# keillernogueira/dynamic-rs-segmentation

Hardware: AMD Instinct MI355X
Metric: training patches/sec dilated_grsl_rate8 64x64x5 (higher is better)
Workload: dtype f32; 1 GPU; dilated_grsl_rate8 (Dilated8Pooling) training step, single_fixed 64x64, 5-band synthetic 2048x2048 tile, global batch 128 (crop+augment+normalise, fwd, loss, bwd, momentum, confusion); global_batch=128, patch=64, bands=5, classes=6, parallelism=dp1, sync_bn=True, rccl_ranks_observed=1

## Files before the change

dynamic-rs-segmentation_amd/_lib.py:

```python
import ctypes as C
import os

_HERE = os.path.dirname(os.path.abspath(__file__))
LIB_PATH = os.path.join(_HERE, "libdrs_hip.so")
DEV_LIB_PATH = os.path.join(_HERE, "libdrs_hip_dev.so")

_p, _i, _f, _d = C.c_void_p, C.c_int, C.c_float, C.c_double
_sz, _u64 = C.c_size_t, C.c_ulonglong

SIGNATURES = {
    "drs_conv_mtile": (_i, [_i]),
    "drs_conv_forward": (_i, [_p, _i, _i, _i, _i, _i, _p, _p, _i, _i, _i, _i, _i, _p, _i, _i, _i, _p, _p]),
    "drs_conv_workspace_floats": (_sz, [_i]),
    "drs_conv_halo_skip": (_i, [_i, _i, _i, _i, _i, _i, _i]),
    "drs_conv_executed_ksteps": (_i, [_i, _i, _i, _i, _i, _i, _i, _p, _p]),
    "drs_conv_forward_ws": (_i, [_p, _i, _i, _i, _i, _i, _p, _p, _i, _i, _i, _i, _i, _p, _i, _i, _i, _p, _p, _sz, _p]),
    "drs_conv_wgrad_splits": (_i, [_i, _i, _i, _i, _i]),
    "drs_conv_wgrad": (_i, [_p, _i, _i, _i, _i, _i, _p, _i, _i, _i, _i, _i, _i, _i, _i, _i, _p, _p, _p]),
    "drs_filter_flip_transpose": (_i, [_p, _p, _i, _i, _i, _p]),
    "drs_filter_pad_cin": (_i, [_p, _p, _i, _i, _i, _i, _p]),
    "drs_split_conv_mtile": (_i, [_i]),
    "drs_split_terms": (_i, [_p, _sz, _i, _p, _p]),
    "drs_filter_split": (_i, [_p, _i, _i, _i, _i, _i, _p, _p, _p]),
    "drs_conv_forward_split": (_i, [_p, _i, _i, _i, _i, _i, _p, _p, _i, _i, _i, _i, _i, _p, _i, _i, _i, _p, _i, _p]),
# ... 73 lines not shown
    "drs_net_receptive_field": (_i, [_p, C.POINTER(_i), C.POINTER(_i)]),
    "drs_net_receptive_field_gated": (_i, [_p, C.POINTER(_i), C.POINTER(_i)]),
    "drs_net_se_info": (_i, [_p, _i, C.c_char_p, _i, C.POINTER(_i), C.POINTER(_i), C.POINTER(_i)]),
    "drs_net_type_name": (_i, [_i, C.c_char_p, _i, C.POINTER(_i)]),
    "drs_net_num_variables": (_i, [_p]),
    "drs_net_variable_info": (_i, [_p, _i, C.c_char_p, _i, C.POINTER(_sz), C.POINTER(_sz), C.POINTER(_i), C.POINTER(_i)]),
    "drs_params_get": (_i, [_p, C.c_char_p, C.c_char_p, _p, _sz, _p]),
    "drs_params_set": (_i, [_p, C.c_char_p, C.c_char_p, _p, _sz, _p]),
    "drs_grad_buffer": (_i, [_p, C.POINTER(_p), C.POINTER(_sz)]),
    "drs_net_global_step": (C.c_longlong, [_p, C.c_longlong]),
    "drs_net_learning_rate": (_f, [_p, _f]),
    "drs_net_set_comm": (_i, [_p, _i, _i, _p, _p, _p]),
    "drs_rccl_bind_library": (_i, [C.c_char_p]),
    "drs_rccl_available": (_i, []),
    "drs_rccl_form": (_i, []),
    "drs_rccl_unique_id": (_i, [_p]),
    "drs_rccl_comm_create": (_i, [_i, _i, _p, C.POINTER(_p)]),
    "drs_rccl_comm_destroy": (_i, [_p]),
    "drs_rccl_all_reduce": (_i, [_p, _p, C.c_size_t, _i, _p]),
    "drs_net_set_rccl": (_i, [_p, _i, _i, _p, _p, _p]),
    "drs_train_step": (_i, [_p, _i, _i, _f, _i, _d, _p]),
    "drs_forward": (_i, [_p, _i, _i, _i, _i, _p]),
    "drs_apply_update": (_i, [_p, _f, _p]),
    "drs_forward_staged": (_i, [_p, _i, _i, _i, _p, _i, _i, _p]),
    "drs_net_se_gate_finish": (_i, [_p, _i, _d, _p]),
    "drs_net_set_two_streams": (_i, [_p, _i]),
    "drs_net_set_class_weights": (_i, [_p, _p, _i]),
    "drs_net_get_class_weights": (_i, [_p, _p, _i, C.POINTER(_i)]),
    "drs_net_set_focal_gamma": (_i, [_p, _f]),
    "drs_net_get_focal_gamma": (_i, [_p, C.POINTER(_f)]),
    "drs_net_timing": (_i, [_p, _i]),
    "drs_net_num_timing_kinds": (_i, []),
    "drs_net_timing_summary": (_i, [_p, _i, C.c_char_p, _i, C.POINTER(_i), C.POINTER(_d), C.POINTER(_d)]),
}
ALLREDUCE_FN = C.CFUNCTYPE(_i, _p, _p, _sz, _i, _i, _p)
WAIT_FN = C.CFUNCTYPE(_i, _p, _i, _p)
WANT_LOGITS, WITH_LABELS, USE_ACC_MASK, USE_LOSS_MASK, NO_UPDATE = 1, 2, 4, 8, 16


DEV_SIGNATURES = {
    "drs_debug_skip_taps": (_i, [_i]), "drs_debug_conv_variant": (_i, [_i]), "drs_debug_conv_wide192": (_i, [_i]),
    "drs_debug_conv_splitk": (_i, [_i]), "drs_debug_conv_hybrid": (_i, [_i]), "drs_debug_conv_sk_order": (_i, [_i]), "drs_debug_conv_prio": (_i, [_i]),
    "drs_debug_conv_sk_geometry": (_i, [_i, _i, _i, _p]), "drs_debug_conv_trace": (_i, [_p]), "drs_debug_conv_lpt": (_i, [_i]), "drs_debug_conv_order": (_i, [_i] * 7 + [_p, _i]),
    "drs_debug_conv_image_tiles": (_i, [_i]), "drs_debug_conv_order_image": (_i, [_i] * 7 + [_p, _i]),
    "drs_debug_wgrad_variant": (_i, [_i]), "drs_debug_wgrad_seg": (_i, [_i]), "drs_debug_wgrad_balance": (_i, [_i]), "drs_debug_wgrad_target": (_i, [_i]),
    "drs_debug_wgrad_len": (_i, [_i]), "drs_debug_wgrad_minchunks": (_i, [_i]), "drs_debug_wgrad_prio": (_i, [_i]), "drs_debug_cls_variant": (_i, [_i]), "drs_debug_slide_blocks": (_i, [_i]), "drs_debug_slide_minrows": (_i, [_i]), "drs_debug_slide_rowpad": (_i, [_i]), "drs_debug_chain_mode": (_i, [_i]), "drs_debug_jitter": (_i, [C.c_ulonglong]), "drs_debug_wg_stream_prio": (_i, [_i]), "drs_debug_reductions_on_chain": (_i, [_i]), "drs_debug_wgrad_schedule": (_i, [_i, _i, _i]), "drs_debug_variant": (_i, [_i]),
    "drs_debug_wgrad_cut": (_i, [_i] * 7 + [_p, _i, _p, _p]),
}


class DrsError(RuntimeError):
    pass


_lib = None
_dev = None


def _open(path, signatures):
    if not os.path.isfile(path):
        raise DrsError("HIP library not built: %s is missing (run dynamic-rs-segmentation_amd/csrc/build.sh "
                       "or __graft_entry__.build()); there is no CPU fallback" % path)
    import torch
    lib = C.CDLL(path)
    for name, (res, args) in signatures.items():
        fn = getattr(lib, name)
        fn.restype = res
        fn.argtypes = args
    return lib


def load():
    global _lib
    if _lib is None:
        _lib = _open(LIB_PATH, SIGNATURES)
    return _lib


class _Dev(object):
# ... 40 lines not shown
```

dynamic-rs-segmentation_amd/csrc/conv_mfma.hip:

```cpp
#include "drs_common.hpp"
#include <algorithm>
#include <cstdlib>
#include <map>
#include <mutex>
#include <numeric>
#include <tuple>
#include <vector>

namespace {

constexpr int BK = 32;
constexpr int LDA = BK + 4;

struct ConvArgs {
  const float* in; int S, P, ld_in, coff_in;
  int M;
  const float* w;
  const float* bias;
  float* out; int ld_out, coff_out;
  float* stats;
  int k, rate, pad, Cin, Cout;
  int accumulate;
  int skip_halo;
  float rcpS, rcpSS;
// ... 1210 lines not shown
  if (W > cap) {
    if (g_conv_splitk <= 0) return plain;
    W = cap; if (G < W || T == tiles) G = W;
  }
  return SkGeom{(int)G, (int)W, (int)T};
}

void conv_lpt_setup(ConvArgs& a, int BM, int mt, int nt, int W) {
  a.lpt_T = 0; a.lpt_ta = a.lpt_tb = a.lpt_P = 0;
  if (W || !g_conv_lpt || drs_g_skip_halo_taps == 0) return;
  const int S2 = a.S * a.S, T = S2 % BM == 0 ? S2 / BM : 0, nblk = mt * nt;
  if (T < 2 || BM % a.S != 0 || nblk % 8 != 0 || (nblk / 8) % (T * nt) != 0) return;
  const int rows = BM / a.S;
  auto full = [&](int t) {
    const int y0 = t * rows, y1 = y0 + rows - 1;
    const int lo = a.pad - y1 > 0 ? (a.pad - y1 + a.rate - 1) / a.rate : 0;
    int hi = (a.S - 1 - y0 + a.pad) / a.rate + 1;
    hi = hi < a.k ? hi : a.k;
    return lo == 0 && hi == a.k;
  };
  int ta = 0, tb = T;
  while (ta < T && !full(ta)) ++ta;
  while (tb > ta && !full(tb - 1)) --tb;
  bool ok = ta < tb;
  for (int t = ta; ok && t < tb; ++t) ok = full(t);
  if (ok && (ta > 0 || tb < T)) { a.lpt_T = T; a.lpt_ta = ta; a.lpt_tb = tb; a.lpt_P = nblk / 8 / (T * nt); a.skip_halo = 1; }
}

int g_conv_image_tiles = -1;

int conv_image_tiles_rule(int k, int rate, int cin, int cout, int B, int S) {
  if (B != 128 || S != 64) return 0;
  struct Row { int k, rate, cin, cout; };
  static const Row gains[] = {{4, 3, 64, 128},
                              {4, 4, 128, 128},
                              {3, 5, 128, 192}, {3, 5, 192, 128},
                              {3, 6, 192, 192},
                              {3, 7, 192, 256}, {3, 7, 256, 192},
                              {3, 8, 256, 256}};
  for (const Row& r : gains)
    if (r.k == k && r.rate == rate && r.cin == cin && r.cout == cout) return 7;
  return 0;
}

int conv_image_tiles_g(int B, int S, int k, int rate, int cin, int cout) {
  const int g = g_conv_image_tiles < 0 ? conv_image_tiles_rule(k, rate, cin, cout, B, S) : g_conv_image_tiles;
  if (g < 4 || g > 7 || k < 2 || cin < BK || cin % BK || g_conv_variant == 0) return 0;
  if (B % (1 << g) || S % (128 >> g)) return 0;
  return g;
}

inline int image_tile_taps(int mt, int S, int k, int rate, int pad, int g) {
  int y, x0, ul, uh, vl, vh;
  image_tile_pos(mt, S, g, y, x0);
  live_taps_image_tile(y, x0, 128 >> g, S, k, rate, pad, ul, uh, vl, vh);
  return (uh - ul) * (vh - vl);
}

std::vector<int> conv_image_order(int B, int S, int k, int rate, int pad, int g) {
  const int mt = B * S * S / 128;
  std::vector<int> taps(mt), sorted(mt), order(mt);
  for (int i = 0; i < mt; ++i) taps[i] = image_tile_taps(i, S, k, rate, pad, g);
  std::iota(sorted.begin(), sorted.end(), 0);
  std::stable_sort(sorted.begin(), sorted.end(), [&](int x, int y) { return taps[x] > taps[y]; });
  if (mt % 8) return sorted;
  const int per = mt / 8;
  for (int c = 0; c < 8; ++c)
    for (int j = 0; j < per; ++j) order[c * per + j] = sorted[j * 8 + c];
  return order;
}

const int* conv_image_order_device(int B, int S, int k, int rate, int pad, int g) {
  static std::mutex mu;
  static std::map<std::tuple<int, int, int, int, int, int, int>, const int*> cache;
  int dev = 0;
  if (hipGetDevice(&dev) != hipSuccess) return nullptr;
  std::lock_guard<std::mutex> lock(mu);
  const auto key = std::make_tuple(dev, B, S, k, rate, pad, g);
  const auto it = cache.find(key);
  if (it != cache.end()) return it->second;
  const std::vector<int> order = conv_image_order(B, S, k, rate, pad, g);
  int* d = nullptr;
  if (hipMalloc((void**)&d, order.size() * sizeof(int)) != hipSuccess) return nullptr;
  if (hipMemcpy(d, order.data(), order.size() * sizeof(int), hipMemcpyHostToDevice) != hipSuccess) { (void)hipFree(d); return nullptr; }
  cache[key] = d;
  return d;
}

template <int BM, int BN, int WM, int WN>
// ... 342 lines not shown
  const int mt = (int)((M + 127) / 128), nt = cout / bn;
  const int W = sk_geometry(mt * nt, k * k * (cin / 32), bn, drs_conv_workspace_floats(cout)).G;
  if (W) return 0;
  conv_lpt_setup(a, 128, mt, nt, 0);
  return a.skip_halo;
}

int drs_conv_executed_ksteps(int B, int S, int k, int rate, int pad_before, int cin, int cout, long long* executed, long long* total) {
  const long long M = (long long)B * S * S;
  if (B < 1 || S < 1 || M >= (1 << 24) || cout < 32 || cout % 32 || cin < 1 || k < 1 || rate < 1 || !executed || !total) return DRS_ERR_ARG;
  const int bn = pick_conv_tile(cout, cin), bm = bn >= 64 ? 128 : 256;
  const int mt = (int)((M + bm - 1) / bm), nt = cout / bn;
  const long long cpt = cin < 32 ? 1 : cin / 32;
  *total = *executed = cin < 32 ? (long long)mt * nt * ((k * k * cin + 31) / 32) : (long long)mt * nt * k * k * cpt;
  if (cin < 32 || cin % 32) return DRS_OK;
  const int g = conv_plain_image_g(B, S, k, rate, cin, cout);
  long long taps = 0;
  if (g) {
    if (drs_g_skip_halo_taps == 0) return DRS_OK;
    for (int i = 0; i < mt; ++i) taps += image_tile_taps(i, S, k, rate, pad_before, g);
  } else {
    if (!drs_conv_halo_skip(B, S, k, rate, pad_before, cin, cout)) return DRS_OK;
    for (int i = 0; i < mt; ++i) {
      const int p0 = i * bm, p1 = (int)(p0 + bm < M ? p0 + bm : M) - 1;
      int y0 = (p0 % (S * S)) / S, y1 = (p1 % (S * S)) / S;
      if (p0 / (S * S) != p1 / (S * S)) { y0 = 0; y1 = S - 1; }
      int lo = pad_before - y1 > 0 ? (pad_before - y1 + rate - 1) / rate : 0, hi = (S - 1 - y0 + pad_before) / rate + 1;
      hi = hi < k ? hi : k;
      if (lo >= hi) { lo = 0; hi = k; }
      taps += (hi - lo) * k;
    }
  }
  *executed = taps * nt * cpt;
  return DRS_OK;
}

int drs_conv_forward_ws(const float* in, int B, int S, int P, int ld_in, int coff_in, const float* w, const float* bias,
                        int k, int rate, int pad_before, int cin, int cout, float* out, int ld_out, int coff_out,
                        int accumulate, float* stats_partial, float* workspace, size_t workspace_floats, void* stream) {
  if (!in || !w || !out || (cin % 32 && cin != 8 && cin != 16) || cout % 32 || k < 1 || rate < 1 || P < pad_before) return DRS_ERR_ARG;
  if (B < 1 || S < 1 || cin < 8 || cout < 32 || pad_before < 0 || !drs_prod_below(1LL << 31, {k, k, cin, cout})) return DRS_ERR_ARG;
  if (coff_in < 0 || ld_in < coff_in + cin || coff_out < 0 || ld_out < coff_out + cout) return DRS_ERR_ARG;
  if (cin < 32 && (ld_in % 4 || coff_in % 4)) return DRS_ERR_ARG;
  if (accumulate && stats_partial) return DRS_ERR_ARG;
  if (P < (long long)(k - 1) * rate - pad_before) return DRS_ERR_ARG;
  const long long M = (long long)B * S * S;
  if (M <= 0 || M >= (1 << 24)) return DRS_ERR_ARG;
  if ((long long)B * (S + 2 * P) * (S + 2 * P) * ld_in >= (1LL << 30)) return DRS_ERR_ARG;
  ConvArgs a;
  a.in = in; a.S = S; a.P = P; a.ld_in = ld_in; a.coff_in = coff_in; a.M = (int)M;
  a.w = w; a.bias = bias; a.out = out; a.ld_out = ld_out; a.coff_out = coff_out; a.stats = stats_partial;
  a.k = k; a.rate = rate; a.pad = pad_before; a.Cin = cin; a.Cout = cout; a.accumulate = accumulate;
  a.rcpS = 1.0f / (float)S; a.rcpSS = 1.0f / (float)(S * S);
  a.skip_halo = drs_skip_halo_taps_fwd(M, cout);
  a.sk_slab = nullptr; a.sk_W = 0; a.sk_nks = 0; a.sk_U = 0; a.sk_T = a.sk_tiles = a.sk_G = a.sk_order = 0; a.prio = 0;
  a.lpt_T = a.lpt_ta = a.lpt_tb = a.lpt_P = 0;
  a.img_g = 0; a.img_order = nullptr;
#ifdef DRS_DEV
  a.trace = g_conv_trace;
#endif
  hipStream_t st = (hipStream_t)stream;
  if (!workspace) workspace_floats = 0;
  switch (pick_conv_tile(cout, cin)) {
    case 192: return launch_conv_dma<128, 192, 2, 2>(a, workspace, workspace_floats, st);
    case 128: return launch_conv<128, 128, 2, 2>(a, workspace, workspace_floats, st);
    case 64:  return launch_conv<128, 64, 2, 2>(a, workspace, workspace_floats, st);
// ... 83 lines not shown
```

dynamic-rs-segmentation_amd/csrc/engine.hip:

```cpp
#include "drs_common.hpp"
#include "../../include/drs.h"

#include <algorithm>
#include <cmath>
#include <cstdio>
#include <cstdlib>
#include <cstring>
#include <map>
#include <string>
#include <vector>

__attribute__((visibility("hidden"))) int drs_step_prep(const StepPrepArgs& a, hipStream_t stream);
__attribute__((visibility("hidden"))) int drs_rccl_all_reduce_sum(void* comm, void* ptr, size_t count, int dtype, hipStream_t stream);

namespace {

struct ConvRow { const char* name; int k, cin, cout, rate, kdim; };
enum Topo { CHAIN = 0, DENSE = 1, SQUEEZE = 2 };
struct NetTable {
  const char* net_type;
  float alpha;
  int max_pool;
  int avg_pool[8];
  Topo topo;
// ... 370 lines not shown

constexpr size_t MAX_RECS = 1 << 16;
struct Timed {
  drs_net* n; hipStream_t st; int kind; TimeRec rec; bool on;
  static bool take(drs_net* n, hipEvent_t* e) {
    if (!n->pool_events.empty()) { *e = n->pool_events.back(); n->pool_events.pop_back(); return true; }
    return hipEventCreate(e) == hipSuccess;
  }
  Timed(drs_net* n_, hipStream_t st_, int kind_, double work) : n(n_), st(st_), kind(kind_), on(n_->timing && n_->recs.size() < MAX_RECS) {
    if (!on) return;
    rec.kind = kind; rec.work = work;
    if (!take(n, &rec.e0)) { on = false; return; }
    if (!take(n, &rec.e1)) { n->pool_events.push_back(rec.e0); on = false; return; }
    (void)hipEventRecord(rec.e0, st);
  }
  ~Timed() {
    if (!on) return;
    (void)hipEventRecord(rec.e1, st);
    n->recs.push_back(rec);
  }
};

#define DRS_TRY(expr) do { const int rc_ = (expr); if (rc_ != DRS_OK) return rc_; } while (0)

#ifdef DRS_DEV
__global__ void jitter_kernel(long long ticks) {
  const long long t0 = wall_clock64();
  while (wall_clock64() - t0 < ticks) __builtin_amdgcn_s_sleep(32);
}
unsigned long long g_jitter_state = 0;
int g_wg_stream_prio = 2;
int g_wg_streams = 1, g_wg_defer = 0;
int g_reductions_on_chain = 0;
inline void jitter(hipStream_t s) {
  if (!g_jitter_state) return;
  g_jitter_state = g_jitter_state * 6364136223846793005ull + 1442695040888963407ull;
  const unsigned r = (unsigned)(g_jitter_state >> 36);
  if (!(r & 1)) return;
  const unsigned span = ((r >> 1) & 7) == 0 ? 400000u : 15000u;
  hipLaunchKernelGGL(jitter_kernel, dim3(1), dim3(64), 0, s, (long long)((r >> 4) % span));
}
#define DRS_JITTER(s) jitter(s)
#else
#define DRS_JITTER(s) do { } while (0)
#endif

inline hipError_t stream_at_priority(hipStream_t* s, int prio) {
  (void)hipGetLastError();
  if (hipStreamCreateWithPriority(s, hipStreamNonBlocking, prio) == hipSuccess) return hipSuccess;
  (void)hipGetLastError();
  return hipStreamCreateWithFlags(s, hipStreamNonBlocking);
}

inline bool collectives(const drs_net* n) { return n->world > 1 || n->allreduce != nullptr || n->rccl_small != nullptr; }

constexpr size_t SMALL_BYTES = 16384;
constexpr size_t MAX_SLABS = 32;

int all_reduce(drs_net* n, int kind, void* ptr, size_t count, int dtype, int async, hipStream_t st, int* handle, bool big_only = false) {
  static const size_t esz[4] = {4, 8, 1, 4};
  if (handle) *handle = -1;
  if (!collectives(n)) return DRS_OK;
  const double bytes = (double)(count * esz[dtype]);
  if (n->rccl_small) {
    if (n->rccl_inline) { Timed t(n, st, kind, bytes); return drs_rccl_all_reduce_sum(n->rccl_small, ptr, count, dtype, st); }
    const bool small = !n->rccl_big || (!(big_only && async) && count * esz[dtype] <= SMALL_BYTES);
    if (!async) { Timed t(n, st, kind, bytes); return drs_rccl_all_reduce_sum(small ? n->rccl_small : n->rccl_big, ptr, count, dtype, st); }
    if (n->comm_in_flight >= n->comm_ring) return DRS_ERR_ARG;
    ++n->comm_in_flight;
    const int h = n->comm_next;
    n->comm_next = (h + 1) % n->comm_ring;
    hipStream_t side = small ? n->small_stream : n->comm_stream;
    if (hipEventRecord(n->comm_events[2 * h], st) != hipSuccess) return DRS_ERR_HIP;
    if (hipStreamWaitEvent(side, n->comm_events[2 * h], 0) != hipSuccess) return DRS_ERR_HIP;
    {
      Timed t(n, side, kind, bytes);
      DRS_TRY(drs_rccl_all_reduce_sum(small ? n->rccl_small : n->rccl_big, ptr, count, dtype, side));
    }
// ... 122 lines not shown
    } else if (L.pool == 2) {
      float* act = P.act;
      { Timed t(n, st, K_BN_FWD, M * L.cout * 8.0);
        DRS_TRY(drs_bn_act_pool_forward(z, B, S, L.cout, mr, n->alpha, 0, act, 0, L.cout, 0, nullptr, st)); }
      Timed t(n, st, K_AVG_FWD, M * L.cout * 8.0);
      DRS_TRY(drs_avg_pool_forward(act, B, S, L.cout, L.avg_k, outp, out.P, out.C, L.dst_coff, st));
      n->halo_ok[L.dst] = -1;
    } else {
      const bool whole = out.C == L.cout && L.dst_coff == 0;
      const long long key = ((long long)B << 20) | S;
      const int hz = (mx && whole && n->halo_ok[L.dst] == key) ? 2 : 0;
      n->halo_ok[L.dst] = (mx && whole) ? key : -1;
      Timed t(n, st, K_BN_FWD, M * L.cout * ((training && mx) ? 9.0 : 8.0));
      if (fold_finish)
        DRS_TRY(drs_bn_finish_act_pool_forward(sums, count, mr, mm, mv, BN_DECAY, n->bessel, z, B, S, L.cout, n->alpha, 1 | hz, outp, out.P, out.C,
                                               L.dst_coff, idx, st));
      else
        DRS_TRY(drs_bn_act_pool_forward(z, B, S, L.cout, mr, n->alpha, (mx ? 1 : 0) | hz, outp, out.P, out.C, L.dst_coff, idx, st));
    }
  }
  return DRS_OK;
}

bool check_bs(const drs_net* n, int B, int S) { return B >= 1 && S >= 1 && B <= n->b_max && S <= n->s_max; }

}

extern "C" {

#ifdef DRS_DEV
int drs_debug_jitter(unsigned long long seed) { g_jitter_state = seed; return 0; }
int drs_debug_wg_stream_prio(int arm) { const int old = g_wg_stream_prio; if (arm >= 0) g_wg_stream_prio = arm; return old; }
int drs_debug_reductions_on_chain(int on) { const int old = g_reductions_on_chain; if (on >= 0) g_reductions_on_chain = on; return old; }
int drs_debug_wgrad_schedule(int layer_slabs, int streams, int defer) {
  if (layer_slabs >= 0) g_wg_layer_slabs = layer_slabs;
  if (streams >= 1) g_wg_streams = streams;
  if (defer >= 0) g_wg_defer = defer;
  return 0;
}
#endif

int drs_net_create(const char* net_type, int channels, int num_classes, float weight_decay, int b_max, int s_max, int bessel_moving_var,
                   float lr_decay_factor, drs_net_t** out) {
  if (!out) return DRS_ERR_ARG;
  *out = nullptr;
  const NetTable* t = find_table(net_type);
  if (!t || channels < 1 || channels > 32 || num_classes < 1 || num_classes > 8 || b_max < 1 || s_max < 1) return DRS_ERR_ARG;
  if ((long long)b_max * s_max * s_max >= (1 << 24)) return DRS_ERR_ARG;
  drs_net* n = nullptr;
  try {
    n = new drs_net();
    n->table = t; n->channels = channels; n->K = num_classes; n->wd = weight_decay; n->b_max = b_max; n->s_max = s_max;
    n->bessel = bessel_moving_var ? 1 : 0; n->lr_decay = lr_decay_factor; n->global_step = 0;
    n->world = 1; n->rank = 0; n->allreduce = nullptr; n->wait = nullptr; n->comm_user = nullptr; n->timing = false;
    n->rccl_small = n->rccl_big = nullptr; n->comm_stream = n->small_stream = nullptr; n->own_comm_stream = false; n->comm_next = 0;
    n->rccl_inline = false; n->rccl_buckets = false; n->comm_ring = 0; n->comm_in_flight = 0;
    for (auto& e : n->ev_bucket) e = nullptr;
    n->wg_stream = nullptr;
    n->two_stream_mode = -1;
    build_plan(n);
    if (n->slabs.size() > MAX_SLABS) { delete n; return DRS_ERR_ARG; }
    list_buffers(n);
    n->halo_ok.assign(n->slabs.size(), -1);
  } catch (...) {
    delete n;
    return DRS_ERR_HIP;
// ... 588 lines not shown
    if (L.se >= 0) {
      const SeBlock& s = n->se[L.se];
      Timed t(n, st, K_SE_BWD, M * L.cout * 16.0);
      DRS_TRY(drs_se_backward(gcur, out.C, L.dst_coff, q.se_act, q.se_s, q.se_e1, q.se_e2, params + s.w1, params + s.w2, B, S, L.cout, s.R, P.gpool,
                              grads + s.w1, grads + s.b1, grads + s.w2, grads + s.b2, P.se_scratch, st));
      gsrc = P.gpool; ldg = L.cout; cg = 0;
    } else if (L.pool == 2) {
      Timed t(n, st, K_AVG_BWD, M * L.cout * 8.0);
      DRS_TRY(drs_avg_pool_backward(gcur, out.C, L.dst_coff, B, S, L.cout, L.avg_k, P.gpool, st));
      gsrc = P.gpool; ldg = L.cout; cg = 0;
    }
    float* z = q.z;
    float* mr = q.mean_rstd;
    {
      Timed t(n, st, K_BN_BWD_REDUCE, M * L.cout * (mx ? 13.0 : 12.0));
      DRS_TRY(drs_bn_backward_reduce(gsrc, ldg, cg, z, mx ? q.idx : nullptr, B, S, L.cout, mr, n->alpha, mx ? 1 : 0, gxh,
                                     partial, st));
    }
    const bool means_form = !collectives(n);
    if (means_form) DRS_TRY(drs_stats_reduce_means(partial, drs_bn_backward_rows(B, S, L.cout, mx ? 1 : 0), L.cout, n_bn, sums, bwd_means, st));
    else DRS_TRY(drs_stats_reduce(partial, drs_bn_backward_rows(B, S, L.cout, mx ? 1 : 0), L.cout, sums, nullptr, st));
    int h_bn;
    DRS_TRY(all_reduce(n, K_AR_SYNCBN, sums, 2 * (size_t)L.cout, F64, two ? 0 : 1, st, &h_bn));
    if (deferred >= 0 && (defer == 0 || defer == 3)) DRS_TRY(filter_gradient(deferred));
    DRS_TRY(wait_handles(n, &h_bn, 1, st));
    float* gz = gzb[two ? (i & 1) : 0];
#ifdef DRS_DEV
    if (xs) gz = q.gzL;
#endif
    if (two && !xs && i + 2 < nL && hipStreamWaitEvent(st, n->ev_wg[i & 1], 0) != hipSuccess) return DRS_ERR_HIP;
    if (two) DRS_JITTER(st);
    {
      Timed t(n, st, K_BN_BWD_APPLY, M * L.cout * 12.0);
      if (means_form) DRS_TRY(drs_bn_backward_apply_means(gxh, z, B, S, L.cout, mr, bwd_means, gz, L.halo, L.cout, 0, st));
      else DRS_TRY(drs_bn_backward_apply(gxh, z, B, S, L.cout, mr, sums, n_bn, gz, L.halo, L.cout, 0, st));
    }
#ifdef DRS_DEV
    if (xs && defer != 3 && hipEventRecord(n->ev_gzL[i], st) != hipSuccess) return DRS_ERR_HIP;
#endif
    if (two && !xs && hipEventRecord(n->ev_gz[i & 1], st) != hipSuccess) return DRS_ERR_HIP;
    if (two) DRS_JITTER(st);
    if (L.src != 0) {
      const Slab& in = n->slabs[L.src];
      const int acc = written[L.src] ? 1 : 0;
      written[L.src] = 1;
      Timed t(n, st, K_CONV_DGRAD, 2.0 * M * L.k * L.k * L.cin * L.cout);
      DRS_TRY(drs_conv_forward_ws(gz, B, S, L.halo, L.cout, 0, q.wt, nullptr, L.k, L.rate, L.pad_a, L.cout, L.cin,
                                  q.gact_in, in.C, 0, acc, nullptr, P.conv_ws, P.conv_ws_floats, st));
    }
#ifdef DRS_DEV
    if (xs && defer == 3 && hipEventRecord(n->ev_gzL[i], st) != hipSuccess) return DRS_ERR_HIP;
#endif
    deferred = i;
  }
#ifdef DRS_DEV
  if (xs) {
    if (defer == 1 || defer == 2) {
      if (hipEventRecord(n->ev_chain_end, st) != hipSuccess) return DRS_ERR_HIP;
      for (int i = nL - 1; i >= 0; --i) DRS_TRY(filter_gradient(i));
    } else {
      DRS_TRY(filter_gradient(deferred));
    }
    for (int j = 0; j < std::min(NS, nL); ++j)
      if (hipStreamWaitEvent(st, n->ev_wgS[j], 0) != hipSuccess) return DRS_ERR_HIP;
  } else
#endif
  {
  DRS_TRY(filter_gradient(deferred));
// ... 53 lines not shown
```

dynamic-rs-segmentation_amd/csrc/pointwise.hip:

```cpp
#include "drs_common.hpp"
#include <cfloat>
#include <cmath>
#include <type_traits>

namespace {

constexpr float BN_EPS = 0.001f;

__device__ __forceinline__ float act(float x, float alpha) { return fmaxf(alpha * x, x); }

constexpr int COLSUM_BLOCKS = 32;

__global__ void colsum_l1_kernel(const float* __restrict__ in, int nrows, int ncols, double* __restrict__ scratch) {
  __shared__ double sh[4][64];
  const int tx = threadIdx.x & 63, ty = threadIdx.x >> 6;
  const int c = blockIdx.x * 64 + tx;
  const int rpb = (nrows + COLSUM_BLOCKS - 1) / COLSUM_BLOCKS;
  const int r0 = blockIdx.y * rpb;
  int r1 = r0 + rpb;
  r1 = r1 < nrows ? r1 : nrows;
  double s = 0.0;
  if (c < ncols)
    for (int r = r0 + ty; r < r1; r += 4) s += (double)in[(size_t)r * ncols + c];
  sh[ty][tx] = s;
// ... 647 lines not shown
    gpre2[(size_t)b * C + c] = g;
  }
  __syncthreads();
  for (int j = threadIdx.x; j < R; j += blockDim.x) {
    float a = 0.f;
    for (int c = 0; c < C; ++c) a += sm[c] * w2[(size_t)j * C + c];
    a = e1[(size_t)b * R + j] > 0.f ? a : 0.f;
    sm[C + j] = a;
    gpre1[(size_t)b * R + j] = a;
  }
  __syncthreads();
  for (int c = threadIdx.x; c < C; c += blockDim.x) {
    float a = 0.f;
    for (int j = 0; j < R; ++j) a += sm[C + j] * w1[(size_t)c * R + j];
    gs[(size_t)b * C + c] = a * inv_hw;
  }
}

__global__ void se_fc_wgrad_kernel(const float* __restrict__ u, const float* __restrict__ v, int B, int rows, int cols,
                                   float* __restrict__ dw, float* __restrict__ db) {
  const int e = blockIdx.x * blockDim.x + threadIdx.x;
  if (e >= (rows + 1) * cols) return;
  const int i = e / cols, j = e - i * cols;
  float a = 0.f;
  if (i < rows) {
    for (int b = 0; b < B; ++b) a += u[(size_t)b * rows + i] * v[(size_t)b * cols + j];
    dw[e] = a;
  } else {
    for (int b = 0; b < B; ++b) a += v[(size_t)b * cols + j];
    db[j] = a;
  }
}

__global__ void bn_bwd_apply_kernel(const float* __restrict__ gxh, const float* __restrict__ z, int B, int S, int C,
                                    const float* __restrict__ mean_rstd, const double* __restrict__ sums, double count,
                                    ActView out, int hp) {
  DRS_CHAIN_PRIO();
  extern __shared__ __attribute__((aligned(16))) float coef[];
  for (int c = threadIdx.x; c < C; c += blockDim.x) {
    coef[c] = mean_rstd[2 * c];
    coef[C + c] = mean_rstd[2 * c + 1];
    coef[2 * C + c] = (float)(sums[2 * c] / count);
    coef[3 * C + c] = (float)(sums[2 * c + 1] / count);
  }
  __syncthreads();
  const int CQ = C >> 2;
  const int Sp = S + 2 * out.P;
  const int e = blockIdx.x * blockDim.x + threadIdx.x;
  if (e >= Sp * CQ) return;
  const int xx = e / CQ, cq = e - xx * CQ;
  const int b = blockIdx.y / Sp, yy = blockIdx.y - b * Sp;
  const size_t dst = ((size_t)(b * Sp + yy) * Sp + xx) * out.ld + out.coff + cq * 4;
  const int y = yy - out.P, x = xx - out.P;
  if (y < 0 || y >= S || x < 0 || x >= S) {
    view_store4(out, dst, f32x4{0.f, 0.f, 0.f, 0.f});
    return;
  }
  const size_t pix = ((size_t)b * S + y) * S + x;
  const f32x4 gv = *reinterpret_cast<const f32x4*>(gxh + pix * C + cq * 4);
  const f32x4 zv = *reinterpret_cast<const f32x4*>(z + pix * C + cq * 4);
  const f32x4 mu = *reinterpret_cast<const f32x4*>(&coef[cq * 4]);
  const f32x4 rs = *reinterpret_cast<const f32x4*>(&coef[C + cq * 4]);
  const f32x4 m1 = *reinterpret_cast<const f32x4*>(&coef[2 * C + cq * 4]);
  const f32x4 m2 = *reinterpret_cast<const f32x4*>(&coef[3 * C + cq * 4]);
  f32x4 o;
#pragma unroll
  for (int j = 0; j < 4; ++j) {
    const float xh = (zv[j] - mu[j]) * rs[j];
    o[j] = rs[j] * (gv[j] - m1[j] - xh * m2[j]);
  }
  view_store4(out, dst, o);
}

__global__ void bn_bwd_apply_means_kernel(const float* __restrict__ gxh, const float* __restrict__ z, int B, int S, int C,
                                          const float* __restrict__ mean_rstd, const float* __restrict__ means, ActView out, int hp) {
  DRS_CHAIN_PRIO();
  const int CQ = C >> 2;
  const int Sp = S + 2 * out.P;
  const int e = blockIdx.x * blockDim.x + threadIdx.x;
  if (e >= Sp * CQ) return;
  const int xx = e / CQ, cq = e - xx * CQ;
  const int b = blockIdx.y / Sp, yy = blockIdx.y - b * Sp;
  const size_t dst = ((size_t)(b * Sp + yy) * Sp + xx) * out.ld + out.coff + cq * 4;
  const int y = yy - out.P, x = xx - out.P;
  if (y < 0 || y >= S || x < 0 || x >= S) {
    view_store4(out, dst, f32x4{0.f, 0.f, 0.f, 0.f});
    return;
  }
  const size_t pix = ((size_t)b * S + y) * S + x;
  const f32x4 gv = *reinterpret_cast<const f32x4*>(gxh + pix * C + cq * 4);
  const f32x4 zv = *reinterpret_cast<const f32x4*>(z + pix * C + cq * 4);
  const f32x4 mr0 = *reinterpret_cast<const f32x4*>(mean_rstd + cq * 8), mr1 = *reinterpret_cast<const f32x4*>(mean_rstd + cq * 8 + 4);
  const f32x4 mm0 = *reinterpret_cast<const f32x4*>(means + cq * 8), mm1 = *reinterpret_cast<const f32x4*>(means + cq * 8 + 4);
  const float mu[4] = {mr0[0], mr0[2], mr1[0], mr1[2]}, rs[4] = {mr0[1], mr0[3], mr1[1], mr1[3]};
  const float m1[4] = {mm0[0], mm0[2], mm1[0], mm1[2]}, m2[4] = {mm0[1], mm0[3], mm1[1], mm1[3]};
  f32x4 o;
#pragma unroll
  for (int j = 0; j < 4; ++j) {
    const float xh = (zv[j] - mu[j]) * rs[j];
    o[j] = rs[j] * (gv[j] - m1[j] - xh * m2[j]);
  }
  view_store4(out, dst, o);
}

struct ClsArgs {
  ActView feat; int C, K, M;
  const float* w;
  const float* bias;
  const unsigned char* labels;
  const unsigned char* loss_mask;
  const unsigned char* acc_mask;
  float inv_n;
  float* logits;
  unsigned char* pred;
  float* gfeat; int ld_g, coff_g;
  float* dw_partial;
  float* db_partial;
  double* loss_partial;
// ... 923 lines not shown
  const int r = bn_bwd_rows_per_block(M);
  return (int)((M + r - 1) / r);
}

int drs_bn_backward_reduce(const float* ga, int ld_ga, int coff_ga, const float* z, const unsigned char* argmax, int B, int S,
                           int C, const float* mean_rstd, float alpha, int pool, float* gxhat, float* partial, void* stream) {
  if (!ga || !z || !mean_rstd || !gxhat || !partial || C % 4 || (pool && !argmax)) return DRS_ERR_ARG;
  const int CQ = C / 4;
  if (CQ > 256) return DRS_ERR_ARG;
  if (!batch_ok(B, S, 0) || !unit_ok(alpha) || !drs_slice_ok(ld_ga, coff_ga, C, 4)) return DRS_ERR_ARG;
  if (pool && slide_ok(C)) {
    const SlideCfg c = slide_cfg(B, S, C);
    const size_t xchg = (size_t)2 * (c.TX + 2) * CQ * 20, redu = (size_t)c.TX * C * 2 * sizeof(float);
    const size_t shm = xchg > redu ? xchg : redu;
    DRS_LAUNCH(bn_bwd_reduce_slide_kernel, dim3(c.ncol, B * c.nstrips), dim3(c.TX * CQ), shm, (hipStream_t)stream, ga, ld_ga, coff_ga, z,
               argmax, B, S, C, mean_rstd, alpha, gxhat, partial, c.nstrips, c.rps, S + g_slide_rowpad, chain_hp());
    return DRS_LAUNCH_CHECK();
  }
  const int PT = 256 / CQ;
  const int nblk = drs_bn_backward_rows(B, S, C, 0);
  const int rpb = bn_bwd_rows_per_block((long long)B * S * S);
  const size_t shm = (size_t)PT * C * 2 * sizeof(float);
  if (pool)
    DRS_LAUNCH(bn_bwd_reduce_kernel<true>, dim3(nblk), dim3(CQ * PT), shm, (hipStream_t)stream, ga, ld_ga, coff_ga, z,
               argmax, B, S, C, mean_rstd, alpha, gxhat, partial, rpb, chain_hp());
  else
    DRS_LAUNCH(bn_bwd_reduce_kernel<false>, dim3(nblk), dim3(CQ * PT), shm, (hipStream_t)stream, ga, ld_ga, coff_ga, z,
               argmax, B, S, C, mean_rstd, alpha, gxhat, partial, rpb, chain_hp());
  return DRS_LAUNCH_CHECK();
}

static int bn_backward_apply_impl(const float* gxhat, const float* z, int B, int S, int C, const float* mean_rstd,
                                  const double* sums, double count, float* gz, int P_out, int ld_out, int coff_out,
                                  unsigned short* terms, int nterms, void* stream) {
  if (!gxhat || !z || !mean_rstd || !sums || (!gz && !terms) || C % 4 || C > 1024) return DRS_ERR_ARG;
  if (terms && ((nterms != 2 && nterms != 3) || (ld_out & 31) || (coff_out & 31))) return DRS_ERR_ARG;
  if (!batch_ok(B, S, P_out) || !count_ok(count) || !drs_slice_ok(ld_out, coff_out, C, 4)) return DRS_ERR_ARG;
  const int Sp = S + 2 * P_out;
  const int per_row = Sp * (C / 4);
  dim3 grid((per_row + 255) / 256, B * Sp);
  ActView v = mkview(gz, S, P_out, ld_out, coff_out);
  v.terms = terms; v.nt = terms ? nterms : 0;
  DRS_LAUNCH(bn_bwd_apply_kernel, grid, dim3(256), (size_t)4 * C * sizeof(float), (hipStream_t)stream, gxhat, z, B, S, C, mean_rstd, sums,
             count, v, chain_hp());
  return DRS_LAUNCH_CHECK();
}

int drs_bn_backward_apply(const float* gxhat, const float* z, int B, int S, int C, const float* mean_rstd, const double* sums,
                          double count, float* gz, int P_out, int ld_out, int coff_out, void* stream) {
  if (!gz) return DRS_ERR_ARG;
  return bn_backward_apply_impl(gxhat, z, B, S, C, mean_rstd, sums, count, gz, P_out, ld_out, coff_out, nullptr, 0, stream);
}

int drs_bn_backward_apply_means(const float* gxhat, const float* z, int B, int S, int C, const float* mean_rstd, const float* means,
                                float* gz, int P_out, int ld_out, int coff_out, void* stream) {
  if (!gxhat || !z || !mean_rstd || !means || !gz || C % 4 || C > 1024) return DRS_ERR_ARG;
  if (!batch_ok(B, S, P_out) || !drs_slice_ok(ld_out, coff_out, C, 4)) return DRS_ERR_ARG;
  const int Sp = S + 2 * P_out;
  const int per_row = Sp * (C / 4);
  DRS_LAUNCH(bn_bwd_apply_means_kernel, dim3((per_row + 255) / 256, B * Sp), dim3(256), 0, (hipStream_t)stream, gxhat, z, B, S, C, mean_rstd,
             means, mkview(gz, S, P_out, ld_out, coff_out), chain_hp());
  return DRS_LAUNCH_CHECK();
}

int drs_bn_backward_apply_terms(const float* gxhat, const float* z, int B, int S, int C, const float* mean_rstd,
                                const double* sums, double count, float* gz, int P_out, int ld_out, int coff_out,
                                unsigned short* terms, int nterms, void* stream) {
  if (!terms) return DRS_ERR_ARG;
  return bn_backward_apply_impl(gxhat, z, B, S, C, mean_rstd, sums, count, gz, P_out, ld_out, coff_out, terms, nterms, stream);
}

int drs_classifier_rows(int B, int S) {
  const long long M = (long long)B * S * S;
  const long long n = (M + 63) / 64;
  return (int)(n < 1 ? 1 : (n > 1024 ? 1024 : n));
}

int g_cls_variant = 1;

#ifdef DRS_DEV
int drs_debug_slide_blocks(int v) { const int old = g_slide_blocks; if (v >= 0) g_slide_blocks = v; return old; }
int drs_debug_slide_rowpad(int v) { const int old = g_slide_rowpad; if (v >= 0) g_slide_rowpad = v; return old; }
int drs_debug_slide_minrows(int v) { const int old = g_slide_minrows; if (v >= 1) g_slide_minrows = v; return old; }
int drs_debug_cls_variant(int v) { const int old = g_cls_variant; if (v >= 0) g_cls_variant = v; return old; }
#endif

int drs_classifier_loss_focal(const float* feat, int B, int S, int P, int ld, int coff, int C, int K, const float* w,
                              const float* bias, const unsigned char* labels, const unsigned char* loss_mask,
                              const unsigned char* acc_mask, float inv_n, const float* class_weights, float focal_gamma,
                              float* logits, unsigned char* pred, float* gfeat, int ld_g, int coff_g, float* dw_partial,
                              float* db_partial, double* loss_partial, unsigned int* conf, void* stream) {
  if (!feat || !w || !bias || K < 1 || K > 8 || C < 64 || C % 64 || C / 64 > 7) return DRS_ERR_ARG;
  if (B < 1 || S < 1 || P < 0 || !std::isfinite(inv_n) || inv_n < 0.f) return DRS_ERR_ARG;
  if (!std::isfinite(focal_gamma) || focal_gamma < 0.f || focal_gamma > 8.f) return DRS_ERR_ARG;
  const long long M = (long long)B * S * S;
  if (M <= 0 || M >= (1 << 24)) return DRS_ERR_ARG;
  if (labels && !loss_partial) return DRS_ERR_ARG;
  if (gfeat && (!dw_partial || !db_partial || !labels)) return DRS_ERR_ARG;
  if (ld % 4 || coff % 4 || (gfeat && (ld_g % 4 || coff_g % 4))) return DRS_ERR_ARG;
  if (!drs_slice_ok(ld, coff, C, 4) || (gfeat && !drs_slice_ok(ld_g, coff_g, C, 4))) return DRS_ERR_ARG;
  if ((long long)B * (S + 2LL * P) * (S + 2LL * P) * ld >= (1LL << 30)) return DRS_ERR_ARG;
  bool wt = false;
// ... 243 lines not shown
```

include/drs.h:

```cpp
#ifndef DRS_H_
#define DRS_H_
#include <stddef.h>

#ifdef __cplusplus
extern "C" {
#endif

#define DRS_OK 0
#define DRS_ERR_ARG 1
#define DRS_ERR_HIP 2

int drs_conv_mtile(int cout);
size_t drs_conv_workspace_floats(int cout);
int drs_conv_halo_skip(int B, int S, int k, int rate, int pad_before, int cin, int cout);
int drs_conv_executed_ksteps(int B, int S, int k, int rate, int pad_before, int cin, int cout, long long* executed, long long* total);
int drs_conv_forward_ws(const float* in, int B, int S, int P, int ld_in, int coff_in, const float* w, const float* bias,
                        int k, int rate, int pad_before, int cin, int cout, float* out, int ld_out, int coff_out,
                        int accumulate, float* stats_partial, float* workspace, size_t workspace_floats, void* stream);
int drs_conv_forward(const float* in, int B, int S, int P, int ld_in, int coff_in, const float* w, const float* bias,
                     int k, int rate, int pad_before, int cin, int cout, float* out, int ld_out, int coff_out,
                     int accumulate, float* stats_partial, void* stream);

int drs_conv_wgrad_splits(int B, int S, int k, int cin, int cout);
int drs_conv_wgrad(const float* x, int B, int S, int Px, int ld_x, int coff_x, const float* g, int Pg, int ld_g,
// ... 171 lines not shown
int drs_net_num_variables(const drs_net_t* net);
int drs_net_variable_info(const drs_net_t* net, int index, char* name, int name_cap, size_t* offset, size_t* count, int* shape4, int* in_bn);
int drs_params_get(drs_net_t* net, const char* name, const char* slot, float* host_dst, size_t count, void* stream);
int drs_params_set(drs_net_t* net, const char* name, const char* slot, const float* host_src, size_t count, void* stream);
int drs_grad_buffer(drs_net_t* net, float** dev_ptr, size_t* count);
long long drs_net_global_step(drs_net_t* net, long long set_to);
float drs_net_learning_rate(const drs_net_t* net, float lr0);
int drs_net_set_comm(drs_net_t* net, int world, int rank, drs_allreduce_fn allreduce, drs_wait_fn wait, void* user);
#define DRS_RCCL_FORM_INLINE 1
#define DRS_RCCL_FORM_ASYNC 2
#define DRS_RCCL_FORM_BUCKETS 3
int drs_rccl_form(void);
int drs_rccl_bind_library(const char* path);
int drs_rccl_available(void);
int drs_rccl_unique_id(unsigned char* id128);
int drs_rccl_comm_create(int world, int rank, const unsigned char* id128, void** comm);
int drs_rccl_comm_destroy(void* comm);
int drs_rccl_all_reduce(void* comm, void* dev_ptr, size_t count, int dtype, void* stream);
int drs_net_set_rccl(drs_net_t* net, int world, int rank, void* comm_small, void* comm_big, void* comm_stream);
int drs_train_step(drs_net_t* net, int B, int S, float lr0, int flags, double global_pixels, void* stream);
int drs_forward(drs_net_t* net, int B, int S, int flags, int ignore_label, void* stream);
int drs_apply_update(drs_net_t* net, float lr0, void* stream);
int drs_forward_staged(drs_net_t* net, int B, int S, int stage, const int* boxes, int n_boxes, int flags, void* stream);
int drs_net_se_gate_finish(drs_net_t* net, int index, double count, void* stream);
int drs_net_set_two_streams(drs_net_t* net, int mode);
int drs_net_set_class_weights(drs_net_t* net, const float* host_w, int K);
int drs_net_get_class_weights(const drs_net_t* net, float* host_w, int K_cap, int* is_set);
int drs_net_set_focal_gamma(drs_net_t* net, float gamma);
int drs_net_get_focal_gamma(const drs_net_t* net, float* gamma);
int drs_net_timing(drs_net_t* net, int enable);
int drs_net_num_timing_kinds(void);
int drs_net_timing_summary(drs_net_t* net, int kind, char* name, int name_cap, int* launches, double* ms, double* work);

int drs_components(const unsigned char* map, int h, int w, int connectivity, int* label, unsigned int* size, void* stream);
size_t drs_sieve_scratch_bytes(int h, int w);
int drs_sieve_round(const unsigned char* map_in, const int* label, const unsigned int* size, int h, int w, int K, const int* min_size,
                    void* scratch, unsigned char* map_out, unsigned int* counters, void* stream);
int drs_component_census(const unsigned char* map, const int* label, const unsigned int* size, int h, int w, int K,
                         unsigned long long* table, void* stream);

#ifdef __cplusplus
}
#endif
#endif
```

include/drs_dev.h:

```cpp
#ifndef DRS_DEV_H_
#define DRS_DEV_H_
#ifdef __cplusplus
extern "C" {
#endif

int drs_debug_skip_taps(int v);
int drs_debug_conv_variant(int v);
int drs_debug_conv_wide192(int v);
int drs_debug_conv_lpt(int v);
int drs_debug_conv_order(int B, int S, int k, int rate, int pad_before, int cin, int cout, int* out, int cap);
int drs_debug_conv_image_tiles(int g);
int drs_debug_conv_order_image(int B, int S, int k, int rate, int pad_before, int cin, int cout, int* out, int cap);
int drs_debug_conv_trace(void* dev_buffer);
int drs_debug_conv_splitk(int v);
int drs_debug_conv_hybrid(int v);
int drs_debug_conv_sk_order(int v);
int drs_debug_conv_prio(int v);
int drs_debug_conv_sk_geometry(int tiles, int nks, int bn, int* out3);
int drs_debug_wgrad_variant(int v);
int drs_debug_wgrad_seg(int v);
int drs_debug_wgrad_balance(int v);
int drs_debug_wgrad_target(int v);
int drs_debug_wgrad_len(int v);
int drs_debug_wgrad_minchunks(int v);
int drs_debug_wgrad_prio(int v);
int drs_debug_slide_blocks(int v);
int drs_debug_slide_minrows(int v);
int drs_debug_jitter(unsigned long long seed);
int drs_debug_wg_stream_prio(int arm);
int drs_debug_reductions_on_chain(int on);
int drs_debug_wgrad_schedule(int layer_slabs, int streams, int defer);
int drs_debug_chain_mode(int v);
int drs_debug_slide_rowpad(int v);
int drs_debug_cls_variant(int v);
int drs_debug_variant(int v);
int drs_debug_wgrad_cut(int B, int S, int k, int rate, int pad_before, int cin, int cout, int* out, int cap, int* out_tile_splits,
                        int* out_tile_rows);

#ifdef __cplusplus
}
#endif
#endif
```

Baseline: 2702 patches/s.

## Skip zeroing gradient halo in BN backward when data-grad conv never reads it

Adds a query that decides whether the data-gradient conv, using image tiles with halo-tap skipping, ever touches the padded border of its input. When it does not, BN backward apply launches an interior-only kernel variant that skips writing zeros to the halo, which saves grid work and stores. It also adds one more layer shape to the image-tile rule table. The risk is that the halo is left stale, which is only safe if every consumer really skips it.

New measurement: 2708 patches/s, median of 6. About the same (+0.2%).

```diff
diff --git a/dynamic-rs-segmentation_amd/_lib.py b/dynamic-rs-segmentation_amd/_lib.py
--- a/dynamic-rs-segmentation_amd/_lib.py
+++ b/dynamic-rs-segmentation_amd/_lib.py
@@ -129,6 +129,9 @@
     "drs_net_timing": (_i, [_p, _i]),
     "drs_net_num_timing_kinds": (_i, []),
     "drs_net_timing_summary": (_i, [_p, _i, C.c_char_p, _i, C.POINTER(_i), C.POINTER(_d), C.POINTER(_d)]),
+    "drs_conv_reads_input_halo": (_i, [_i, _i, _i, _i, _i, _i, _i, _p]),
+    "drs_bn_backward_apply_interior": (_i, [_p, _p, _i, _i, _i, _p, _p, _d, _p, _i, _i, _i, _p]),
+    "drs_bn_backward_apply_means_interior": (_i, [_p, _p, _i, _i, _i, _p, _p, _p, _i, _i, _i, _p]),
 }
 ALLREDUCE_FN = C.CFUNCTYPE(_i, _p, _p, _sz, _i, _i, _p)
 WAIT_FN = C.CFUNCTYPE(_i, _p, _i, _p)
@@ -141,7 +144,7 @@
     "drs_debug_conv_sk_geometry": (_i, [_i, _i, _i, _p]), "drs_debug_conv_trace": (_i, [_p]), "drs_debug_conv_lpt": (_i, [_i]), "drs_debug_conv_order": (_i, [_i] * 7 + [_p, _i]),
     "drs_debug_conv_image_tiles": (_i, [_i]), "drs_debug_conv_order_image": (_i, [_i] * 7 + [_p, _i]),
     "drs_debug_wgrad_variant": (_i, [_i]), "drs_debug_wgrad_seg": (_i, [_i]), "drs_debug_wgrad_balance": (_i, [_i]), "drs_debug_wgrad_target": (_i, [_i]),
-    "drs_debug_wgrad_len": (_i, [_i]), "drs_debug_wgrad_minchunks": (_i, [_i]), "drs_debug_wgrad_prio": (_i, [_i]), "drs_debug_cls_variant": (_i, [_i]), "drs_debug_slide_blocks": (_i, [_i]), "drs_debug_slide_minrows": (_i, [_i]), "drs_debug_slide_rowpad": (_i, [_i]), "drs_debug_chain_mode": (_i, [_i]), "drs_debug_jitter": (_i, [C.c_ulonglong]), "drs_debug_wg_stream_prio": (_i, [_i]), "drs_debug_reductions_on_chain": (_i, [_i]), "drs_debug_wgrad_schedule": (_i, [_i, _i, _i]), "drs_debug_variant": (_i, [_i]),
+    "drs_debug_wgrad_len": (_i, [_i]), "drs_debug_wgrad_minchunks": (_i, [_i]), "drs_debug_wgrad_prio": (_i, [_i]), "drs_debug_cls_variant": (_i, [_i]), "drs_debug_slide_blocks": (_i, [_i]), "drs_debug_slide_minrows": (_i, [_i]), "drs_debug_slide_rowpad": (_i, [_i]), "drs_debug_chain_mode": (_i, [_i]), "drs_debug_jitter": (_i, [C.c_ulonglong]), "drs_debug_wg_stream_prio": (_i, [_i]), "drs_debug_reductions_on_chain": (_i, [_i]), "drs_debug_gz_halo": (_i, [_i]),"drs_debug_wgrad_schedule": (_i, [_i, _i, _i]), "drs_debug_variant": (_i, [_i]),
     "drs_debug_wgrad_cut": (_i, [_i] * 7 + [_p, _i, _p, _p]),
 }
 
diff --git a/dynamic-rs-segmentation_amd/csrc/conv_mfma.hip b/dynamic-rs-segmentation_amd/csrc/conv_mfma.hip
--- a/dynamic-rs-segmentation_amd/csrc/conv_mfma.hip
+++ b/dynamic-rs-segmentation_amd/csrc/conv_mfma.hip
@@ -1266,7 +1266,7 @@
 int conv_image_tiles_rule(int k, int rate, int cin, int cout, int B, int S) {
   if (B != 128 || S != 64) return 0;
   struct Row { int k, rate, cin, cout; };
-  static const Row gains[] = {{4, 3, 64, 128},
+  static const Row gains[] = {{4, 3, 64, 128}, {4, 3, 128, 64},
                               {4, 4, 128, 128},
                               {3, 5, 128, 192}, {3, 5, 192, 128},
                               {3, 6, 192, 192},
@@ -1289,6 +1289,17 @@
   image_tile_pos(mt, S, g, y, x0);
   live_taps_image_tile(y, x0, 128 >> g, S, k, rate, pad, ul, uh, vl, vh);
   return (uh - ul) * (vh - vl);
+}
+
+inline bool image_tiles_read_halo(int S, int k, int rate, int pad, int g) {
+  if (g != 7 || drs_g_skip_halo_taps == 0) return true;
+  for (int c = 0; c < S; ++c) {
+    int ul, uh, vl, vh;
+    live_taps_image_tile(c, c, 1, S, k, rate, pad, ul, uh, vl, vh);
+    if (ul >= uh || vl >= vh) return true;
+    if (c + ul * rate - pad < 0 || c + (uh - 1) * rate - pad >= S || c + vl * rate - pad < 0 || c + (vh - 1) * rate - pad >= S) return true;
+  }
+  return false;
 }
 
 std::vector<int> conv_image_order(int B, int S, int k, int rate, int pad, int g) {
@@ -1697,6 +1708,14 @@
     }
   }
   *executed = taps * nt * cpt;
+  return DRS_OK;
+}
+
+int drs_conv_reads_input_halo(int B, int S, int k, int rate, int pad_before, int cin, int cout, int* reads) {
+  const long long M = (long long)B * S * S;
+  if (!reads || B < 1 || S < 1 || M >= (1 << 24) || k < 1 || rate < 1 || pad_before < 0) return DRS_ERR_ARG;
+  if ((cin % 32 && cin != 8 && cin != 16) || cin < 8 || cout < 32 || cout % 32 || !drs_prod_below(1LL << 31, {k, k, cin, cout})) return DRS_ERR_ARG;
+  *reads = image_tiles_read_halo(S, k, rate, pad_before, conv_plain_image_g(B, S, k, rate, cin, cout)) ? 1 : 0;
   return DRS_OK;
 }
 
diff --git a/dynamic-rs-segmentation_amd/csrc/engine.hip b/dynamic-rs-segmentation_amd/csrc/engine.hip
--- a/dynamic-rs-segmentation_amd/csrc/engine.hip
+++ b/dynamic-rs-segmentation_amd/csrc/engine.hip
@@ -426,6 +426,7 @@
 int g_wg_stream_prio = 2;
 int g_wg_streams = 1, g_wg_defer = 0;
 int g_reductions_on_chain = 0;
+int g_gz_halo = -1;
 inline void jitter(hipStream_t s) {
   if (!g_jitter_state) return;
   g_jitter_state = g_jitter_state * 6364136223846793005ull + 1442695040888963407ull;
@@ -438,6 +439,16 @@
 #else
 #define DRS_JITTER(s) do { } while (0)
 #endif
+
+inline bool gz_halo_unread(const Layer& L, int B, int S) {
+#ifdef DRS_DEV
+  if (g_gz_halo == 1) return false;
+#endif
+  if (L.src == 0) return true;
+  int reads = 1;
+  if (drs_conv_reads_input_halo(B, S, L.k, L.rate, L.pad_a, L.cout, L.cin, &reads) != DRS_OK) return false;
+  return reads == 0;
+}
 
 inline hipError_t stream_at_priority(hipStream_t* s, int prio) {
   (void)hipGetLastError();
@@ -626,6 +637,7 @@
 int drs_debug_jitter(unsigned long long seed) { g_jitter_state = seed; return 0; }
 int drs_debug_wg_stream_prio(int arm) { const int old = g_wg_stream_prio; if (arm >= 0) g_wg_stream_prio = arm; return old; }
 int drs_debug_reductions_on_chain(int on) { const int old = g_reductions_on_chain; if (on >= 0) g_reductions_on_chain = on; return old; }
+int drs_debug_gz_halo(int v) { const int old = g_gz_halo; if (v == -1 || v == 1) g_gz_halo = v; return old; }
 int drs_debug_wgrad_schedule(int layer_slabs, int streams, int defer) {
   if (layer_slabs >= 0) g_wg_layer_slabs = layer_slabs;
   if (streams >= 1) g_wg_streams = streams;
@@ -1280,8 +1292,9 @@
     if (two) DRS_JITTER(st);
     {
       Timed t(n, st, K_BN_BWD_APPLY, M * L.cout * 12.0);
-      if (means_form) DRS_TRY(drs_bn_backward_apply_means(gxh, z, B, S, L.cout, mr, bwd_means, gz, L.halo, L.cout, 0, st));
-      else DRS_TRY(drs_bn_backward_apply(gxh, z, B, S, L.cout, mr, sums, n_bn, gz, L.halo, L.cout, 0, st));
+      const bool inner = gz_halo_unread(L, B, S);
+      if (means_form) DRS_TRY((inner ? drs_bn_backward_apply_means_interior : drs_bn_backward_apply_means)(gxh, z, B, S, L.cout, mr, bwd_means, gz, L.halo, L.cout, 0, st));
+      else DRS_TRY((inner ? drs_bn_backward_apply_interior : drs_bn_backward_apply)(gxh, z, B, S, L.cout, mr, sums, n_bn, gz, L.halo, L.cout, 0, st));
     }
 #ifdef DRS_DEV
     if (xs && defer != 3 && hipEventRecord(n->ev_gzL[i], st) != hipSuccess) return DRS_ERR_HIP;
diff --git a/dynamic-rs-segmentation_amd/csrc/pointwise.hip b/dynamic-rs-segmentation_amd/csrc/pointwise.hip
--- a/dynamic-rs-segmentation_amd/csrc/pointwise.hip
+++ b/dynamic-rs-segmentation_amd/csrc/pointwise.hip
@@ -703,6 +703,7 @@
   }
 }
 
+template <bool INNER>
 __global__ void bn_bwd_apply_kernel(const float* __restrict__ gxh, const float* __restrict__ z, int B, int S, int C,
                                     const float* __restrict__ mean_rstd, const double* __restrict__ sums, double count,
                                     ActView out, int hp) {
@@ -718,12 +719,14 @@
   const int CQ = C >> 2;
   const int Sp = S + 2 * out.P;
   const int e = blockIdx.x * blockDim.x + threadIdx.x;
-  if (e >= Sp * CQ) return;
-  const int xx = e / CQ, cq = e - xx * CQ;
-  const int b = blockIdx.y / Sp, yy = blockIdx.y - b * Sp;
+  const int W = INNER ? S : Sp;
+  if (e >= W * CQ) return;
+  const int xg = e / CQ, cq = e - xg * CQ;
+  const int b = blockIdx.y / W, yg = blockIdx.y - b * W;
+  const int yy = INNER ? yg + out.P : yg, xx = INNER ? xg + out.P : xg;
   const size_t dst = ((size_t)(b * Sp + yy) * Sp + xx) * out.ld + out.coff + cq * 4;
   const int y = yy - out.P, x = xx - out.P;
-  if (y < 0 || y >= S || x < 0 || x >= S) {
+  if (!INNER && (y < 0 || y >= S || x < 0 || x >= S)) {
     view_store4(out, dst, f32x4{0.f, 0.f, 0.f, 0.f});
     return;
   }
@@ -743,18 +746,21 @@
   view_store4(out, dst, o);
 }
 
+template <bool INNER>
 __global__ void bn_bwd_apply_means_kernel(const float* __restrict__ gxh, const float* __restrict__ z, int B, int S, int C,
                                           const float* __restrict__ mean_rstd, const float* __restrict__ means, ActView out, int hp) {
   DRS_CHAIN_PRIO();
   const int CQ = C >> 2;
   const int Sp = S + 2 * out.P;
   const int e = blockIdx.x * blockDim.x + threadIdx.x;
-  if (e >= Sp * CQ) return;
-  const int xx = e / CQ, cq = e - xx * CQ;
-  const int b = blockIdx.y / Sp, yy = blockIdx.y - b * Sp;
+  const int W = INNER ? S : Sp;
+  if (e >= W * CQ) return;
+  const int xg = e / CQ, cq = e - xg * CQ;
+  const int b = blockIdx.y / W, yg = blockIdx.y - b * W;
+  const int yy = INNER ? yg + out.P : yg, xx = INNER ? xg + out.P : xg;
   const size_t dst = ((size_t)(b * Sp + yy) * Sp + xx) * out.ld + out.coff + cq * 4;
   const int y = yy - out.P, x = xx - out.P;
-  if (y < 0 || y >= S || x < 0 || x >= S) {
+  if (!INNER && (y < 0 || y >= S || x < 0 || x >= S)) {
     view_store4(out, dst, f32x4{0.f, 0.f, 0.f, 0.f});
     return;
   }
@@ -1744,42 +1750,67 @@
 
 static int bn_backward_apply_impl(const float* gxhat, const float* z, int B, int S, int C, const float* mean_rstd,
                                   const double* sums, double count, float* gz, int P_out, int ld_out, int coff_out,
-                                  unsigned short* terms, int nterms, void* stream) {
+                                  unsigned short* terms, int nterms, bool interior, void* stream) {
   if (!gxhat || !z || !mean_rstd || !sums || (!gz && !terms) || C % 4 || C > 1024) return DRS_ERR_ARG;
   if (terms && ((nterms != 2 && nterms != 3) || (ld_out & 31) || (coff_out & 31))) return DRS_ERR_ARG;
   if (!batch_ok(B, S, P_out) || !count_ok(count) || !drs_slice_ok(ld_out, coff_out, C, 4)) return DRS_ERR_ARG;
-  const int Sp = S + 2 * P_out;
-  const int per_row = Sp * (C / 4);
-  dim3 grid((per_row + 255) / 256, B * Sp);
+  const int W = interior ? S : S + 2 * P_out;
+  const int per_row = W * (C / 4);
+  dim3 grid((per_row + 255) / 256, B * W);
   ActView v = mkview(gz, S, P_out, ld_out, coff_out);
   v.terms = terms; v.nt = terms ? nterms : 0;
-  DRS_LAUNCH(bn_bwd_apply_kernel, grid, dim3(256), (size_t)4 * C * sizeof(float), (hipStream_t)stream, gxhat, z, B, S, C, mean_rstd, sums,
-             count, v, chain_hp());
+  if (interior)
+    DRS_LAUNCH(bn_bwd_apply_kernel<true>, grid, dim3(256), (size_t)4 * C * sizeof(float), (hipStream_t)stream, gxhat, z, B, S, C, mean_rstd,
+               sums, count, v, chain_hp());
+  else
+    DRS_LAUNCH(bn_bwd_apply_kernel<false>, grid, dim3(256), (size_t)4 * C * sizeof(float), (hipStream_t)stream, gxhat, z, B, S, C, mean_rstd,
+               sums, count, v, chain_hp());
+  return DRS_LAUNCH_CHECK();
+}
+
+static int bn_backward_apply_means_impl(const float* gxhat, const float* z, int B, int S, int C, const float* mean_rstd, const float* means,
+                                        float* gz, int P_out, int ld_out, int coff_out, bool interior, void* stream) {
+  if (!gxhat || !z || !mean_rstd || !means || !gz || C % 4 || C > 1024) return DRS_ERR_ARG;
+  if (!batch_ok(B, S, P_out) || !drs_slice_ok(ld_out, coff_out, C, 4)) return DRS_ERR_ARG;
+  const int W = interior ? S : S + 2 * P_out;
+  const int per_row = W * (C / 4);
+  dim3 grid((per_row + 255) / 256, B * W);
+  if (interior)
+    DRS_LAUNCH(bn_bwd_apply_means_kernel<true>, grid, dim3(256), 0, (hipStream_t)stream, gxhat, z, B, S, C, mean_rstd, means,
+               mkview(gz, S, P_out, ld_out, coff_out), chain_hp());
+  else
+    DRS_LAUNCH(bn_bwd_apply_means_kernel<false>, grid, dim3(256), 0, (hipStream_t)stream, gxhat, z, B, S, C, mean_rstd, means,
+               mkview(gz, S, P_out, ld_out, coff_out), chain_hp());
   return DRS_LAUNCH_CHECK();
 }
 
 int drs_bn_backward_apply(const float* gxhat, const float* z, int B, int S, int C, const float* mean_rstd, const double* sums,
                           double count, float* gz, int P_out, int ld_out, int coff_out, void* stream) {
   if (!gz) return DRS_ERR_ARG;
-  return bn_backward_apply_impl(gxhat, z, B, S, C, mean_rstd, sums, count, gz, P_out, ld_out, coff_out, nullptr, 0, stream);
+  return bn_backward_apply_impl(gxhat, z, B, S, C, mean_rstd, sums, count, gz, P_out, ld_out, coff_out, nullptr, 0, false, stream);
 }
 
 int drs_bn_backward_apply_means(const float* gxhat, const float* z, int B, int S, int C, const float* mean_rstd, const float* means,
                                 float* gz, int P_out, int ld_out, int coff_out, void* stream) {
-  if (!gxhat || !z || !mean_rstd || !means || !gz || C % 4 || C > 1024) return DRS_ERR_ARG;
-  if (!batch_ok(B, S, P_out) || !drs_slice_ok(ld_out, coff_out, C, 4)) return DRS_ERR_ARG;
-  const int Sp = S + 2 * P_out;
-  const int per_row = Sp * (C / 4);
-  DRS_LAUNCH(bn_bwd_apply_means_kernel, dim3((per_row + 255) / 256, B * Sp), dim3(256), 0, (hipStream_t)stream, gxhat, z, B, S, C, mean_rstd,
-             means, mkview(gz, S, P_out, ld_out, coff_out), chain_hp());
-  return DRS_LAUNCH_CHECK();
+  return bn_backward_apply_means_impl(gxhat, z, B, S, C, mean_rstd, means, gz, P_out, ld_out, coff_out, false, stream);
+}
+
+int drs_bn_backward_apply_interior(const float* gxhat, const float* z, int B, int S, int C, const float* mean_rstd, const double* sums,
+                                   double count, float* gz, int P_out, int ld_out, int coff_out, void* stream) {
+  if (!gz) return DRS_ERR_ARG;
+  return bn_backward_apply_impl(gxhat, z, B, S, C, mean_rstd, sums, count, gz, P_out, ld_out, coff_out, nullptr, 0, true, stream);
+}
+
+int drs_bn_backward_apply_means_interior(const float* gxhat, const float* z, int B, int S, int C, const float* mean_rstd,
+                                         const float* means, float* gz, int P_out, int ld_out, int coff_out, void* stream) {
+  return bn_backward_apply_means_impl(gxhat, z, B, S, C, mean_rstd, means, gz, P_out, ld_out, coff_out, true, stream);
 }
 
 int drs_bn_backward_apply_terms(const float* gxhat, const float* z, int B, int S, int C, const float* mean_rstd,
                                 const double* sums, double count, float* gz, int P_out, int ld_out, int coff_out,
                                 unsigned short* terms, int nterms, void* stream) {
   if (!terms) return DRS_ERR_ARG;
-  return bn_backward_apply_impl(gxhat, z, B, S, C, mean_rstd, sums, count, gz, P_out, ld_out, coff_out, terms, nterms, stream);
+  return bn_backward_apply_impl(gxhat, z, B, S, C, mean_rstd, sums, count, gz, P_out, ld_out, coff_out, terms, nterms, false, stream);
 }
 
 int drs_classifier_rows(int B, int S) {
diff --git a/include/drs.h b/include/drs.h
--- a/include/drs.h
+++ b/include/drs.h
@@ -227,6 +227,13 @@
 int drs_net_num_timing_kinds(void);
 int drs_net_timing_summary(drs_net_t* net, int kind, char* name, int name_cap, int* launches, double* ms, double* work);
 
+int drs_conv_reads_input_halo(int B, int S, int k, int rate, int pad_before, int cin, int cout, int* reads);
+int drs_bn_backward_apply_interior(const float* gxhat, const float* z, int B, int S, int C, const float* mean_rstd,
+                                   const double* sums, double count, float* gz, int P_out, int ld_out, int coff_out,
+                                   void* stream);
+int drs_bn_backward_apply_means_interior(const float* gxhat, const float* z, int B, int S, int C, const float* mean_rstd,
+                                         const float* means, float* gz, int P_out, int ld_out, int coff_out, void* stream);
+
 int drs_components(const unsigned char* map, int h, int w, int connectivity, int* label, unsigned int* size, void* stream);
 size_t drs_sieve_scratch_bytes(int h, int w);
 int drs_sieve_round(const unsigned char* map_in, const int* label, const unsigned int* size, int h, int w, int K, const int* min_size,
diff --git a/include/drs_dev.h b/include/drs_dev.h
--- a/include/drs_dev.h
+++ b/include/drs_dev.h
@@ -29,6 +29,7 @@
 int drs_debug_jitter(unsigned long long seed);
 int drs_debug_wg_stream_prio(int arm);
 int drs_debug_reductions_on_chain(int on);
+int drs_debug_gz_halo(int v);
 int drs_debug_wgrad_schedule(int layer_slabs, int streams, int defer);
 int drs_debug_chain_mode(int v);
 int drs_debug_slide_rowpad(int v);
```
